# facebookresearch/NasRec

Measured on AMD Instinct MI355X. Metric: supernet samples/sec at batch 256 (Criteo-shape), 1/2/4/8 MI355X, higher is better.
Workload: dtype f32

## Files before the change

### nasrec_amd/csrc/gemm_rt.h

```cpp
#pragma once
#include <type_traits>
#include "gemm_tile.h"

struct RtStride {
  int R1, R0, K1, K0;
  bool kcontig;
};

__device__ __forceinline__ RtStride rt_stride(int mode, int ld) {
  if (mode == NASREC_AM_KC) return RtStride{16 * ld, ld, 16, 1, true};
  if (mode == NASREC_AM_RC) return RtStride{16, 1, 16 * ld, ld, false};
  if (mode == NASREC_AM_TOKR) return RtStride{ld, 1, 256, 16, false};
  return RtStride{256, 16, ld, 1, true};
}

__device__ __forceinline__ long rt_offset(const RtStride& s, int r, int k) {
  return (long)(r >> 4) * s.R1 + (long)(r & 15) * s.R0 + (long)(k >> 4) * s.K1 + (long)(k & 15) * s.K0;
}

template <bool KCONTIG, int NT, int TK, int R>
__device__ __forceinline__ void rt_stage_coords(int tid, int it, int& rr, int& kk) {
  if (KCONTIG) {
    kk = 4 * (tid & (TK / 4 - 1));
    rr = tid / (TK / 4) + (NT / (TK / 4)) * it;
  } else {
    rr = 4 * (tid & (R / 4 - 1));
    kk = tid / (R / 4) + (NT / (R / 4)) * it;
  }
}

__device__ __forceinline__ void rt_epilogue_store(int cm, const nasrec_gemm_desc_t& d, const nasrec_gemm_seg_t& sg, int i, int j, float v) {
  if (cm == NASREC_CM_PLAIN)
    epilogue_store<NASREC_CM_PLAIN>(d, sg, i, j, v);
  else
    epilogue_store<NASREC_CM_TOKJ>(d, sg, i, j, v);
}

__device__ __forceinline__ void rt_epilogue_store_col4(int cm, const nasrec_gemm_desc_t& d, const nasrec_gemm_seg_t& sg, int i0, int j, int M, const float (&v4)[4]) {
  if (cm == NASREC_CM_PLAIN)
    epilogue_store_col4<NASREC_CM_PLAIN>(d, sg, i0, j, M, v4);
  else
    epilogue_store_col4<NASREC_CM_TOKJ>(d, sg, i0, j, M, v4);
}

#define GEMM_RT_LDS_FLOATS(TBM, TBN, TK) (((TBM) + (TBN)) * ((TK) + 4) + 128)

template <bool KCA, bool KCB, int NT, int TK, int TBM, int TBN, bool AUX, int RING>
__device__ __forceinline__ void gemm_tile_rt(const nasrec_gemm_desc_t& d, int Mmax, int Nmax, const int bx, const int by, const int bz, float* lds) {
  const int AM = d.amode, BMODE = d.bmode, CM = d.cmode;
  constexpr int LDS_LD = TK + 4;
  constexpr int VA = 4, VB = 4;
  constexpr int NITA = TBM * TK / NT / VA, NITB = TBN * TK / NT / VB;
  static_assert((TBM * TK / NT) % VA == 0 && (TBN * TK / NT) % VB == 0 && TK % 16 == 0 && TBM % 4 == 0 && TBN % 4 == 0, "whole 16-byte pieces");
  constexpr int PER_WAVE = (TBM / 16) * (TBN / 16) / (NT / 64);
  constexpr int WTM = (PER_WAVE >= 2 && TBM >= 32) ? 32 : 16;
  constexpr int WTN = 16 * PER_WAVE / (WTM / 16);
  constexpr int FA = WTM / 16, FB = WTN / 16;
  static_assert(NITA >= 1 && NITB >= 1 && PER_WAVE >= 1 && (TBM / WTM) * (TBN / WTN) == NT / 64, "tile configuration");
  float* As = lds;
  float* Bs = lds + TBM * LDS_LD;
  const int tid = threadIdx.x;
  const int lane = tid & 63, wave = tid >> 6;
  const int wm = wave / (TBN / WTN), wn = wave % (TBN / WTN);
  const int fr = lane & 15, fg = lane >> 4;
  const int S = d.splitk > 1 ? d.splitk : 1;
  const int z = d.zmode ? bz / S : 0;
  const int ks = bz % S;
  const nasrec_gemm_seg_t& s0 = d.seg[z];
  const int M = s0.M, N = s0.N;
  const int m0 = by * TBM, n0 = bx * TBN;
  if (m0 >= M || n0 >= N) return;

  struct SegInfo {
    const float *A, *B, *Ax, *Bx;
    int K, lda, ldb, live;
  };
  static_assert(sizeof(SegInfo) * NASREC_MAX_SEGS <= 128 * sizeof(float), "segment table area");
  SegInfo* sinfo = reinterpret_cast<SegInfo*>(lds + (TBM + TBN) * LDS_LD);
  const bool use_table = !d.zmode && d.nseg > 1;
  if (use_table) {
    if (tid < d.nseg) {
      const nasrec_gemm_seg_t& sg = d.seg[tid];
      sinfo[tid] = SegInfo{sg.A, sg.B, sg.Aaux, sg.Baux, sg.K, sg.lda, sg.ldb, (sg.A != nullptr && sg.K > 0) ? 1 : 0};
    }
    __syncthreads();
  }
  int T = 0;
  if (!use_table) {
    T = (s0.A != nullptr && s0.K > 0) ? (s0.K + TK - 1) / TK : 0;
  } else {
    for (int q = 0; q < d.nseg; ++q)
      if (sinfo[q].live) T += (sinfo[q].K + TK - 1) / TK;
  }
  const int t0 = (int)((long)T * ks / S), t1 = (int)((long)T * (ks + 1) / S);

  f32x4 acc[FA][FB];
#pragma unroll
  for (int a = 0; a < FA; ++a)
#pragma unroll
    for (int b = 0; b < FB; ++b) acc[a][b] = (f32x4){0.f, 0.f, 0.f, 0.f};

  const int cOnes = s0.ones_col;
  const int Ra = (s0.Mvalid > 0 && s0.Mvalid < M) ? s0.Mvalid : M;
  const int Rb = cOnes ? N - 1 : N;
  const bool edgeA = (m0 + TBM > Ra), edgeB = (n0 + TBN > Rb);
  bool rvA[NITA], rvB[NITB];
  int kkA[NITA], kkB[NITB];
#pragma unroll
  for (int it = 0; it < NITA; ++it) {
    int rr;
    rt_stage_coords<KCA, NT, TK, TBM>(tid, it, rr, kkA[it]);
    rvA[it] = (m0 + rr) < Ra;
  }
#pragma unroll
  for (int it = 0; it < NITB; ++it) {
    int rr;
    rt_stage_coords<KCB, NT, TK, TBN>(tid, it, rr, kkB[it]);
    rvB[it] = (n0 + rr) < Rb;
  }

  int fs = z, fkt = t0;
  if (use_table) {
    fs = 0;
    int skip = t0;
    while (fs < d.nseg) {
      const int nt = sinfo[fs].live ? (sinfo[fs].K + TK - 1) / TK : 0;
      if (skip < nt) break;
      skip -= nt;
      ++fs;
    }
    fkt = skip;
  }
  const __amdgpu_buffer_rsrc_t rs_null = __builtin_amdgcn_make_buffer_rsrc(nullptr, 0, 0, 0x00020000);
  __amdgpu_buffer_rsrc_t rsA = rs_null, rsB = rs_null, rsAx = rs_null, rsBx = rs_null;
  bool hasAaux = false, hasBaux = false;
  int cK = 0, seg_tiles = 0;
  int stepA = 0, stepB = 0;
  unsigned voffA[NITA], voffB[NITB];
  unsigned koffA[NITA], koffB[NITB];
  auto load_seg = [&](int sq) {
    auto uptr = [](const float* p) -> const float* {
      const unsigned long long v = (unsigned long long)p;
      const unsigned lo = __builtin_amdgcn_readfirstlane((unsigned)v), hi = __builtin_amdgcn_readfirstlane((unsigned)(v >> 32));
      return (const float*)(((unsigned long long)hi << 32) | lo);
    };
    struct {
      const float *A, *B, *Aaux, *Baux;
      int K, lda, ldb;
    } sg;
    if (use_table) {
      sg = {uptr(sinfo[sq].A), uptr(sinfo[sq].B), uptr(sinfo[sq].Ax), uptr(sinfo[sq].Bx), __builtin_amdgcn_readfirstlane(sinfo[sq].K),
            __builtin_amdgcn_readfirstlane(sinfo[sq].lda), __builtin_amdgcn_readfirstlane(sinfo[sq].ldb)};
    } else {
      const nasrec_gemm_seg_t& g = d.seg[sq];
      sg = {g.A, g.B, g.Aaux, g.Baux, g.K, g.lda, g.ldb};
    }
    const int lda = sg.lda, ldb = sg.ldb;
    const RtStride sa_ = rt_stride(AM, lda), sb_ = rt_stride(BMODE, ldb);
    const int Rb_mem = cOnes ? N - 1 : N;
    const int extA = (M > 0 && sg.K > 0) ? (int)(4 * (rt_offset(sa_, M - 1, sg.K - 1) + 1)) : 0;
    const int extB = (Rb_mem > 0 && sg.K > 0) ? (int)(4 * (rt_offset(sb_, Rb_mem - 1, sg.K - 1) + 1)) : 0;
    rsA = __builtin_amdgcn_make_buffer_rsrc(const_cast<float*>(sg.A), 0, extA, 0x00020000);
    rsB = __builtin_amdgcn_make_buffer_rsrc(const_cast<float*>(sg.B), 0, extB, 0x00020000);
    hasAaux = AUX && sg.Aaux != nullptr;
    hasBaux = AUX && sg.Baux != nullptr;
    rsAx = hasAaux ? __builtin_amdgcn_make_buffer_rsrc(const_cast<float*>(sg.Aaux), 0, extA, 0x00020000) : rs_null;
    rsBx = hasBaux ? __builtin_amdgcn_make_buffer_rsrc(const_cast<float*>(sg.Baux), 0, extB, 0x00020000) : rs_null;
    cK = sg.K;
    seg_tiles = (cK + TK - 1) / TK;
    stepA = (int)(4 * rt_offset(sa_, 0, TK));
    stepB = (int)(4 * rt_offset(sb_, 0, TK));
#pragma unroll
    for (int it = 0; it < NITA; ++it) {
      int rr, kk;
      rt_stage_coords<KCA, NT, TK, TBM>(tid, it, rr, kk);
      koffA[it] = 4u * (unsigned)rt_offset(sa_, 0, kk);
      voffA[it] = 4u * (unsigned)rt_offset(sa_, rvA[it] ? m0 + rr : 0, kk);
    }
#pragma unroll
    for (int it = 0; it < NITB; ++it) {
      int rr, kk;
      rt_stage_coords<KCB, NT, TK, TBN>(tid, it, rr, kk);
      koffB[it] = 4u * (unsigned)rt_offset(sb_, 0, kk);
      voffB[it] = 4u * (unsigned)rt_offset(sb_, rvB[it] ? n0 + rr : 0, kk);
    }
  };

  float ra[RING][NITA][VA], rb[RING][NITB][VB];
  float xa[AUX ? RING : 1][AUX ? NITA : 1][VA], xb[AUX ? RING : 1][AUX ? NITB : 1][VB];
  auto stage_load = [](auto vtag, const __amdgpu_buffer_rsrc_t& rs, int voff, int soff, float* dst) {
    if (decltype(vtag)::value == 4) {
      const f32x4 t = __builtin_bit_cast(f32x4, __builtin_amdgcn_raw_buffer_load_b128(rs, voff, soff, 0));
      dst[0] = t[0], dst[1 % decltype(vtag)::value] = t[1], dst[2 % decltype(vtag)::value] = t[2], dst[3 % decltype(vtag)::value] = t[3];
    } else {
      dst[0] = __builtin_bit_cast(float, __builtin_amdgcn_raw_buffer_load_b32(rs, voff, soff, 0));
    }
  };
  using TagA = std::integral_constant<int, VA>;
  using TagB = std::integral_constant<int, VB>;
  int lim[RING];
  int fetched = t0;
  auto fetch = [&](int slot) {
    const bool live = fetched < t1;
    const int l = live ? cK - fkt * TK : 0;
    lim[slot] = l;
    const __amdgpu_buffer_rsrc_t ua = live ? rsA : rs_null, ub = live ? rsB : rs_null;
    const int sa = fkt * stepA, sb = fkt * stepB;
#pragma unroll
    for (int it = 0; it < NITA; ++it) {
      const int o = (int)((kkA[it] < l) ? voffA[it] : voffA[it] - koffA[it]);
      stage_load(TagA{}, ua, o, sa, ra[slot][it]);
      if (AUX) stage_load(TagA{}, live ? rsAx : rs_null, o, sa, xa[slot][it]);
    }
#pragma unroll
    for (int it = 0; it < NITB; ++it) {
      const int o = (int)((kkB[it] < l) ? voffB[it] : voffB[it] - koffB[it]);
      stage_load(TagB{}, ub, o, sb, rb[slot][it]);
      if (AUX) stage_load(TagB{}, live ? rsBx : rs_null, o, sb, xb[slot][it]);
    }
  };
  auto advance = [&]() {
    ++fetched;
    if (fetched >= t1) return;
    ++fkt;
    if (fkt >= seg_tiles) {
      if (use_table) {
        do {
          ++fs;
        } while (fs < d.nseg && !sinfo[fs].live);
        fkt = 0;
        load_seg(fs);
      }
    }
  };
  auto commit = [&](int slot) {
    const int l = lim[slot];
#pragma unroll
    for (int it = 0; it < NITA; ++it) {
      int rr, kk;
      rt_stage_coords<KCA, NT, TK, TBM>(tid, it, rr, kk);
      float a[VA];
#pragma unroll
      for (int e = 0; e < VA; ++e) {
        a[e] = ra[slot][it][e];
        if (AUX) a[e] = (!hasAaux || xa[slot][it][e] > 0.f) ? a[e] : 0.f;
        if (edgeA) a[e] = (m0 + rr + (KCA ? 0 : e) < Ra) ? a[e] : 0.f;
        a[e] = (kk + (KCA ? e : 0) < l) ? a[e] : 0.f;
      }
      if (KCA) {
        *reinterpret_cast<f32x4*>(&As[rr * LDS_LD + kk]) = (f32x4){a[0], a[1], a[2], a[3]};
      } else {
#pragma unroll
        for (int e = 0; e < VA; ++e) As[(rr + e) * LDS_LD + kk] = a[e];
      }
    }
#pragma unroll
    for (int it = 0; it < NITB; ++it) {
      int rr, kk;
      rt_stage_coords<KCB, NT, TK, TBN>(tid, it, rr, kk);
      float b[VB];
#pragma unroll
      for (int e = 0; e < VB; ++e) {
        b[e] = rb[slot][it][e];
        if (AUX) b[e] = (!hasBaux || xb[slot][it][e] > 0.f) ? b[e] : 0.f;
        if (edgeB) b[e] = (n0 + rr + (KCB ? 0 : e) < Rb) ? b[e] : 0.f;
        const bool kin = kk + (KCB ? e : 0) < l;
        b[e] = kin ? b[e] : 0.f;
        if (cOnes && (n0 + rr + (KCB ? 0 : e) == N - 1)) b[e] = kin ? 1.f : 0.f;
      }
      if (KCB) {
        *reinterpret_cast<f32x4*>(&Bs[rr * LDS_LD + kk]) = (f32x4){b[0], b[1], b[2], b[3]};
      } else {
#pragma unroll
        for (int e = 0; e < VB; ++e) Bs[(rr + e) * LDS_LD + kk] = b[e];
      }
    }
  };
  auto mfma_tile = [&]() {
#pragma unroll
    for (int kb = 0; kb < TK / 16; ++kb) {
      f32x4 af[FA], bf[FB];
#pragma unroll
      for (int a = 0; a < FA; ++a) af[a] = *reinterpret_cast<const f32x4*>(&As[(wm * WTM + a * 16 + fr) * LDS_LD + kb * 16 + 4 * fg]);
#pragma unroll
      for (int b = 0; b < FB; ++b) bf[b] = *reinterpret_cast<const f32x4*>(&Bs[(wn * WTN + b * 16 + fr) * LDS_LD + kb * 16 + 4 * fg]);
#pragma unroll
      for (int j = 0; j < 4; ++j)
#pragma unroll
        for (int a = 0; a < FA; ++a)
#pragma unroll
          for (int b = 0; b < FB; ++b) acc[a][b] = __builtin_amdgcn_mfma_f32_16x16x4f32(af[a][j], bf[b][j], acc[a][b], 0, 0, 0);
    }
  };

  if (t0 < t1) {
    load_seg(fs);
#pragma unroll
// ... 50 lines not shown
```

### nasrec_amd/csrc/worklist.hip

```cpp
#include <stdlib.h>
#include <string.h>

#include <vector>

#include "worklist_body.h"

static int wl_gemm_geometry(const nasrec_gemm_desc_t* g, nasrec_wl_item_t& it, int blob_left) {
  if (g->nseg < 1 || g->nseg > NASREC_MAX_SEGS) return nasrec_set_error(-2, "worklist: gemm nseg=%d", g->nseg);
  const int need = (int)offsetof(nasrec_gemm_desc_t, seg) + g->nseg * (int)sizeof(nasrec_gemm_seg_t);
  if (need > blob_left) return nasrec_set_error(-2, "worklist: truncated gemm descriptor (%d bytes) runs past the blob", need);
  const int nprob = g->zmode ? g->nseg : 1;
  const int S = g->splitk > 1 ? g->splitk : 1;
  if (g->splitk == NASREC_SPLITK_BALANCED) return nasrec_set_error(-2, "worklist: the balanced schedule is a throughput-regime launch");
  if ((it.part == 0) != (S == 1)) return nasrec_set_error(-2, "worklist: gemm part %d with splitk %d", it.part, g->splitk);
  if (S > 1 && !g->workspace) return nasrec_set_error(-3, "worklist: splitk=%d needs a workspace", S);
  int Mmax = 0, Nmax = 0, Kmax = 0;
  long wgs = 0;
  bool aux = false, uniform = true;
  for (int q = 0; q < nprob; ++q) {
    Mmax = g->seg[q].M > Mmax ? g->seg[q].M : Mmax;
    Nmax = g->seg[q].N > Nmax ? g->seg[q].N : Nmax;
    wgs += (long)((g->seg[q].M + 63) / 64) * ((g->seg[q].N + 63) / 64) * S;
  }
  for (int q = 0; q < g->nseg; ++q) {
    const nasrec_gemm_seg_t& s = g->seg[q];
    if (s.A && s.K > Kmax) Kmax = s.K;
    aux = aux || s.Aaux || s.Baux;
    if (!g->zmode && (s.ones_col != g->seg[0].ones_col || s.Mvalid != g->seg[0].Mvalid)) uniform = false;
    if (!g->zmode && s.A && ((s.Aaux != nullptr) != (g->seg[0].Aaux != nullptr) || (s.Baux != nullptr) != (g->seg[0].Baux != nullptr))) uniform = false;
  }
  if (!uniform) return nasrec_set_error(-2, "worklist: k-segments that disagree on row predicates / mask operands take the plain template");
  {
    const bool kca = g->amode == NASREC_AM_KC || g->amode == NASREC_AM_TOKK, kcb = g->bmode == NASREC_AM_KC || g->bmode == NASREC_AM_TOKK;
    if (!kca && kcb) return nasrec_set_error(-2, "worklist: operand binding a=%d b=%d has no body", g->amode, g->bmode);
  }
  if (Mmax <= 0 || Nmax <= 0) {
    it.nblk = 0;
    return 0;
  }
  if (it.part == 2) {
    const int per = (int)(((long)Mmax * Nmax + 255) / 256);
    it.geom[0] = per;
    it.nblk = per * nprob;
    return 0;
  }
  static const bool dense_body = getenv("NASREC_WL_DENSE_BODY") == nullptr || atoi(getenv("NASREC_WL_DENSE_BODY")) != 0;
  if (dense_body && it.part == 0 && !g->zmode && !aux && g->amode == NASREC_AM_KC && g->bmode == NASREC_AM_KC && g->cmode == NASREC_CM_PLAIN) {
    bool plain = true;
    int steps = 0;
    for (int q = 0; q < g->nseg; ++q) {
      const nasrec_gemm_seg_t& s = g->seg[q];
      plain = plain && !s.ones_col && !(s.Mvalid > 0 && s.Mvalid < Mmax);
      plain = plain && (long)Mmax * s.lda + s.K < (1L << 29) && (long)Nmax * s.ldb + s.K < (1L << 29);
      steps += (s.A && s.K > 0) ? (s.K + 15) >> 4 : 1;
    }
    if (plain && steps <= 2 * WL_DENSE_STEPS && (Mmax + 15) / 16 < 0x10000) {
      it.geom[0] = (Nmax + 15) / 16;
      it.geom[1] = (Mmax + 15) / 16 | (((steps + WL_DENSE_STEPS - 1) / WL_DENSE_STEPS) << 16);
      it.geom[2] = WL_TOKS | (3 << 2);
      it.nblk = (it.geom[0] * ((Mmax + 15) / 16) + 3) / 4;
      return 0;
    }
  }
  bool aux_b = false;
// ... 37 lines not shown
    for (int q = 0; q < g->nseg; ++q) {
      const nasrec_gemm_seg_t& s = g->seg[q];
      plain = plain && !s.ones_col && !(s.Mvalid > 0 && s.Mvalid < s.M) && s.N == Nmax && s.K <= 16 * WL_TOKDX_STEPS && s.M > 0;
      TU += (s.M + 15) / 16;
    }
    if (plain) {
      it.geom[0] = TU;
      it.geom[1] = 0;
      it.geom[2] = WL_TOKS | (2 << 2);
      it.nblk = std::min(((Nmax >> 4) * TU + 3) / 4, WL_TOK_MAX_WG);
      return 0;
    }
  }
  int tile, tbm, tbn;
  if (wgs >= GEMM_SKINNY_BELOW) {
    tile = WL_T32x32, tbm = 32, tbn = 32;
  } else {
    long pad64x16 = 0, pad16x64 = 0;
    for (int q = 0; q < nprob; ++q) {
      pad64x16 += (long)((g->seg[q].M + 63) / 64) * 64 * ((g->seg[q].N + 15) / 16) * 16;
      pad16x64 += (long)((g->seg[q].M + 15) / 16) * 16 * ((g->seg[q].N + 63) / 64) * 64;
    }
    static const bool by_padding = getenv("NASREC_WL_TILE_BY_PADDING") == nullptr || atoi(getenv("NASREC_WL_TILE_BY_PADDING")) != 0;
    const bool wide = by_padding && pad64x16 != pad16x64 ? pad64x16 < pad16x64 : Nmax >= Mmax;
    if (wide) {
      tile = WL_T64x16, tbm = 64, tbn = 16;
    } else {
      tile = WL_T16x64, tbm = 16, tbn = 64;
    }
  }
  it.geom[0] = (Nmax + tbn - 1) / tbn;
  it.geom[1] = (Mmax + tbm - 1) / tbm;
  const bool kca_ = g->amode == NASREC_AM_KC || g->amode == NASREC_AM_TOKK, kcb_ = g->bmode == NASREC_AM_KC || g->bmode == NASREC_AM_TOKK;
  it.geom[2] = tile | ((kca_ && kcb_ ? 0 : (kca_ ? 1 : 2)) << 2) | ((aux ? 1 : 0) << 4);
  it.nblk = it.geom[0] * it.geom[1] * nprob * S;
  return 0;
}

static int wl_item_geometry(nasrec_wl_item_t& it, const char* blob, int left, int k, bool& big) {
    it.nblk = 0;
    it.geom[0] = it.geom[1] = it.geom[2] = 0;
#define WL_NEED(T) if ((int)sizeof(T) > left) return nasrec_set_error(-2, "worklist: item %d runs past the blob", k)
    switch (it.kind) {
      case NASREC_OP_GEMM: {
        const int rc = wl_gemm_geometry(reinterpret_cast<const nasrec_gemm_desc_t*>(blob), it, left);
        if (rc) return rc;
        break;
      }
      case NASREC_OP_MHA_FWD:
      case NASREC_OP_MHA_BWD: {
        WL_NEED(nasrec_mha_desc_t);
        const nasrec_mha_desc_t* d = reinterpret_cast<const nasrec_mha_desc_t*>(blob);
        if (d->N < 1 || d->N > MHA_N) return nasrec_set_error(-2, "worklist: mha N=%d out of range [1,%d]", d->N, MHA_N);
        if (it.kind == NASREC_OP_MHA_BWD) {
          if (!d->saved) return nasrec_set_error(-2, "worklist: mha backward needs the state saved by the forward launch");
          big = true;
        }
        it.nblk = d->B;
        break;
      }
      case NASREC_OP_FM_FWD:
      case NASREC_OP_FM_BWD:
        WL_NEED(nasrec_fm_desc_t);
        it.nblk = (reinterpret_cast<const nasrec_fm_desc_t*>(blob)->B + 3) / 4;
        break;
      case NASREC_OP_DOT_TRI_FWD:
      case NASREC_OP_DOT_TRI_BWD: {
// ... 140 lines not shown
  if (!d->dev) return nasrec_set_error(-2, "worklist (device-resident): not prepared");
  if (d->total_blocks < 1) return 0;
  const unsigned* pf = d->pf;
  const unsigned* pm = d->pm;
  if (d->big) {
    hipLaunchKernelGGL(worklist_dev_kernel<true>, dim3((unsigned)d->total_blocks), dim3(256), sizeof(float) * WL_LDS_BIG_FLOATS, st, pf[0], pf[1], pf[2], pf[3],
                       pf[4], pf[5], pm[0], pm[1], pm[2], pm[3], pm[4], pm[5], d->dev);
  } else {
    hipLaunchKernelGGL(worklist_dev_kernel<false>, dim3((unsigned)d->total_blocks), dim3(256), sizeof(float) * WL_LDS_FLOATS, st, pf[0], pf[1], pf[2], pf[3],
                       pf[4], pf[5], pm[0], pm[1], pm[2], pm[3], pm[4], pm[5], d->dev);
  }
  return nasrec_check_launch("worklist (device-resident)");
}

#define PS_SPIN_BUDGET_TICKS 1000000ull

template <bool BIG>
__device__ __forceinline__ void ps_run_item(int it_kind, int it_part, int g0, int g1, int g2, unsigned long long blob, int vb, int nblk, int nwg) {
  float* lds = wl_lds;
  const int tid = threadIdx.x, wave = tid >> 6, lane = tid & 63;
  switch (it_kind) {
    case NASREC_OP_GEMM: {
      if (it_part == 2) {
        for (int u = vb; u < nblk; u += nwg) wl_gemm_second_pass(blob, u, g0);
        break;
      }
      const int cfg = g2;
      if ((cfg & 3) == WL_TOKS && ((cfg >> 2) & 3) == 3 && g1 == 0) wl_dense_small_dx(blob, vb, g0);
      else if ((cfg & 3) == WL_TOKS && ((cfg >> 2) & 3) == 3) wl_dense_small(blob, vb, g0, g1);
      else if ((cfg & 3) == WL_TOKS && ((cfg >> 2) & 3) == 1) wl_token_fwd(blob, vb, g0);
      else if ((cfg & 3) == WL_TOKS) wl_token_dx(blob, vb, g0);
      else if ((cfg >> 4) & 1) {
        for (int u = vb; u < nblk; u += nwg) {
          wl_gemm_bind<true>((cfg >> 2) & 3, cfg & 3, blob, u, g0, g1);
          if (u + nwg < nblk) __syncthreads();
        }
      } else {
        for (int u = vb; u < nblk; u += nwg) {
          wl_gemm_bind<false>((cfg >> 2) & 3, cfg & 3, blob, u, g0, g1);
          if (u + nwg < nblk) __syncthreads();
        }
      }
      break;
    }
    case NASREC_OP_MHA_FWD:
      wl_mha_fwd(blob, vb);
      break;
    case NASREC_OP_MHA_BWD:
      if (BIG) mha_bwd_tok(wl_ref<nasrec_mha_desc_t>(blob), __builtin_amdgcn_readfirstlane(vb), wl_lds);
      break;
    case NASREC_OP_FM_FWD: {
      const nasrec_fm_desc_t& d = wl_ref<nasrec_fm_desc_t>(blob);
      const int b = vb * 4 + wave;
      if (b < d.B) fm_fwd_sample(d, b, lane);
      break;
    }
    case NASREC_OP_FM_BWD: {
      const nasrec_fm_desc_t& d = wl_ref<nasrec_fm_desc_t>(blob);
      const int b = vb * 4 + wave;
      if (b < d.B) fm_bwd_sample(d, b, lane);
      break;
    }
    case NASREC_OP_DOT_TRI_FWD: {
      const nasrec_dot_tri_desc_t& d = wl_ref<nasrec_dot_tri_desc_t>(blob);
      const int b = vb * 4 + wave;
      if (b < d.B) dot_tri_fwd_sample(d, b, lane, lds + wave * (d.k1 * TRI_LD));
      break;
    }
    case NASREC_OP_DOT_TRI_BWD: {
      const nasrec_dot_tri_desc_t& d = wl_ref<nasrec_dot_tri_desc_t>(blob);
      const int b = vb * 4 + wave;
      const int P4 = (d.k1 * (d.k1 - 1) / 2 + 3) & ~3;
// ... 190 lines not shown
```

### nasrec_amd/csrc/worklist_body.h

```cpp
#pragma once
#include "attention_tok.h"
#include "gemm_rt.h"
#include "final_bodies.h"
#include "interact_bodies.h"
#include "dedup_bodies.h"

#define WL_LDS_BIG_FLOATS 9888
#define WL_LDS_FLOATS 7840
static_assert(MHA_TOK_BWD_LDS_FLOATS <= WL_LDS_BIG_FLOATS && MHA_TOK_FWD_LDS_FLOATS <= WL_LDS_FLOATS, "Transformer bodies fit the worklist launches");

#define WL_TK 64
#ifndef WL_AUX_RING2
#define WL_AUX_RING2 0
#endif
enum { WL_TOKS = 0, WL_T32x32 = 1, WL_T64x16 = 2, WL_T16x64 = 3 };

extern __shared__ __attribute__((aligned(16))) float wl_lds[];

template <typename T>
__device__ __forceinline__ const T& wl_ref(unsigned long long addr) {
  const unsigned lo = __builtin_amdgcn_readfirstlane((unsigned)addr), hi = __builtin_amdgcn_readfirstlane((unsigned)(addr >> 32));
  return *(const T*)(const __attribute__((address_space(4))) T*)(((unsigned long long)hi << 32) | lo);
}

template <bool KCA, bool KCB, int TBM, int TBN, bool AUX>
__device__ __forceinline__ void wl_gemm_cfg(unsigned long long blob, int vb_, int gx_, int gy_) {
  constexpr int RING = (AUX && !WL_AUX_RING2) ? 1 : 2;
  const nasrec_gemm_desc_t& g = wl_ref<nasrec_gemm_desc_t>(blob);
  const int vb = __builtin_amdgcn_readfirstlane(vb_), gx = __builtin_amdgcn_readfirstlane(gx_), gy = __builtin_amdgcn_readfirstlane(gy_);
  const int nprob = g.zmode ? g.nseg : 1;
  int Mmax = 0, Nmax = 0;
  for (int q = 0; q < nprob; ++q) {
    Mmax = max(Mmax, g.seg[q].M);
    Nmax = max(Nmax, g.seg[q].N);
  }
  const int bx = vb % gx, by = (vb / gx) % gy, bz = vb / (gx * gy);
  gemm_tile_rt<KCA, KCB, 256, WL_TK, TBM, TBN, AUX, RING>(g, Mmax, Nmax, bx, by, bz, wl_lds);
}

template <bool KCA, bool KCB, bool AUX>
__device__ __forceinline__ void wl_gemm_tile(int tile, unsigned long long off, int vb, int gx, int gy) {
  switch (tile) {
    case WL_T32x32: wl_gemm_cfg<KCA, KCB, 32, 32, AUX>(off, vb, gx, gy); break;
    case WL_T64x16: wl_gemm_cfg<KCA, KCB, 64, 16, AUX>(off, vb, gx, gy); break;
    default: wl_gemm_cfg<KCA, KCB, 16, 64, AUX>(off, vb, gx, gy); break;
  }
}

template <bool AUX>
__device__ __forceinline__ void wl_gemm_bind(int bind, int tile, unsigned long long off, int vb, int gx, int gy) {
  if (bind == 0) wl_gemm_tile<true, true, AUX>(tile, off, vb, gx, gy);
  else if (bind == 1) wl_gemm_tile<true, false, AUX>(tile, off, vb, gx, gy);
  else wl_gemm_tile<false, false, AUX>(tile, off, vb, gx, gy);
}

__device__ __forceinline__ void wl_warm_blob(unsigned long long addr, int bytes) {
  int sink, off;
  asm volatile(
      "s_mov_b32 %1, 0\n"
      "1:\n"
      "s_load_dword %0, %2, %1\n"
      "s_add_u32 %1, %1, 64\n"
      "s_cmp_lt_u32 %1, %3\n"
      "s_cbranch_scc1 1b\n"
      "s_waitcnt lgkmcnt(0)"
      : "=&s"(sink), "=&s"(off)
      : "s"(addr), "s"(bytes)
      : "scc", "memory");
}

#define WL_TOK_DEPTH 4
__device__ __forceinline__ void wl_token_fwd(unsigned long long blob, int vb_, int MT_) {
  const nasrec_gemm_desc_t& g = wl_ref<nasrec_gemm_desc_t>(blob);
  const int vb = __builtin_amdgcn_readfirstlane(vb_), MT = __builtin_amdgcn_readfirstlane(MT_);
  const int lane = threadIdx.x & 63, wave = __builtin_amdgcn_readfirstlane(threadIdx.x >> 6);
  const int e = lane & 15, fg = lane >> 4;
  wl_warm_blob(blob, (int)offsetof(nasrec_gemm_desc_t, seg) + g.nseg * (int)sizeof(nasrec_gemm_seg_t));
  const nasrec_gemm_seg_t& s0 = g.seg[0];
  const int M = s0.M, B = s0.N >> 4;
  const int unit = vb * 4 + wave;
  const int b = unit / MT, mt = unit - b * MT;
  if (b >= B) return;
  const int row = min(mt * 16 + e, M - 1);
  f32x4 acc = {0.f, 0.f, 0.f, 0.f};
  f32x4 fa[WL_TOK_DEPTH];
  float fb[WL_TOK_DEPTH][4];
// ... 275 lines not shown
    for (int q = 1; q < NASREC_WL_MAX_ITEMS; ++q) {
      const unsigned fq = (f[q >> 1] >> (16 * (q & 1))) & 0xffffu, mq = (m[q >> 1] >> (16 * (q & 1))) & 0xffffu;
      if ((unsigned)bid >= fq) {
        k = q;
        it_first = (int)fq;
        meta = mq;
      }
    }
    it_kind = meta & 63;
    it_part = (meta >> 6) & 3;
    it_off = (int)(meta >> 8) * 16;
  } else {
#pragma unroll 1
    while (k + 1 < wl.n && bid >= wl.item[k + 1].first) ++k;
    it_first = wl.item[k].first;
    it_kind = wl.item[k].kind;
    it_part = wl.item[k].part;
    it_off = wl.item[k].off;
  }
  const nasrec_wl_item_t& it = wl.item[k];
  const int vb = bid - it_first;
  const unsigned long long blob = base + offsetof(nasrec_worklist_desc_t, blob) + it_off;
  switch (it_kind) {
    case NASREC_OP_GEMM: {
      if (it_part == 2) {
        wl_gemm_second_pass(blob, vb, it.geom[0]);
        break;
      }
      const int cfg = it.geom[2];
      if ((cfg & 3) == WL_TOKS && ((cfg >> 2) & 3) == 3 && it.geom[1] == 0) wl_dense_small_dx(blob, vb, it.geom[0]);
      else if ((cfg & 3) == WL_TOKS && ((cfg >> 2) & 3) == 3) wl_dense_small(blob, vb, it.geom[0], it.geom[1]);
      else if ((cfg & 3) == WL_TOKS && ((cfg >> 2) & 3) == 1) wl_token_fwd(blob, vb, it.geom[0]);
      else if ((cfg & 3) == WL_TOKS) wl_token_dx(blob, vb, it.geom[0]);
      else if ((cfg >> 4) & 1) wl_gemm_bind<true>((cfg >> 2) & 3, cfg & 3, blob, vb, it.geom[0], it.geom[1]);
      else wl_gemm_bind<false>((cfg >> 2) & 3, cfg & 3, blob, vb, it.geom[0], it.geom[1]);
      break;
    }
    case NASREC_OP_MHA_FWD:
      wl_mha_fwd(blob, vb);
      break;
    case NASREC_OP_MHA_BWD:
      if (BIG) mha_bwd_tok(wl_ref<nasrec_mha_desc_t>(blob), __builtin_amdgcn_readfirstlane(vb), wl_lds);
      break;
    case NASREC_OP_FM_FWD: {
      const nasrec_fm_desc_t& d = wl_ref<nasrec_fm_desc_t>(blob);
      const int b = vb * 4 + wave;
      if (b < d.B) fm_fwd_sample(d, b, lane);
      break;
    }
    case NASREC_OP_FM_BWD: {
      const nasrec_fm_desc_t& d = wl_ref<nasrec_fm_desc_t>(blob);
      const int b = vb * 4 + wave;
      if (b < d.B) fm_bwd_sample(d, b, lane);
      break;
    }
    case NASREC_OP_DOT_TRI_FWD: {
      const nasrec_dot_tri_desc_t& d = wl_ref<nasrec_dot_tri_desc_t>(blob);
      const int b = vb * 4 + wave;
      if (b < d.B) dot_tri_fwd_sample(d, b, lane, lds + wave * (d.k1 * TRI_LD));
      break;
    }
    case NASREC_OP_DOT_TRI_BWD: {
      const nasrec_dot_tri_desc_t& d = wl_ref<nasrec_dot_tri_desc_t>(blob);
      const int b = vb * 4 + wave;
      const int P4 = (d.k1 * (d.k1 - 1) / 2 + 3) & ~3;
      if (b < d.B) dot_tri_bwd_sample(d, b, lane, lds + wave * (d.k1 * TRI_LD), lds + 4 * (d.k1 * TRI_LD) + wave * P4);
      break;
    }
// ... 45 lines not shown
```

### nasrec_amd/schedule.py

```python
import ctypes as C
import os
from typing import List, Tuple

from . import _lib as L

E = 16
MHA_PARAM_FLOATS = [768, 48, 256, 16, 16, 16, 256, 16, 256, 16, 16, 16]


class Acc:
    __slots__ = ("ptr", "width", "stride", "rows", "end")

    def __init__(self, ptr, rows, width_f, ld_f):
        self.ptr = int(ptr)
        self.rows = max(int(rows), 1)
        self.width = int(width_f) * 4
        self.stride = int(ld_f) * 4 if self.rows > 1 else self.width
        if self.stride < self.width:
            self.stride = self.width
        self.end = self.ptr + (self.rows - 1) * self.stride + self.width


def _flat(ptr, n_floats):
    return Acc(ptr, 1, n_floats, n_floats)
# ... 451 lines not shown


SOLO_TILES = int(os.environ.get("NASREC_WL_SOLO_TILES", "256"))


def gemm_capable(d) -> bool:
    if d.splitk == L.SPLITK_BALANCED or d.defer_second_pass or d.nseg < 1 or d.nseg > L.MAX_SEGS:
        return False
    kca, kcb = d.amode in (L.AM_KC, L.AM_TOKK), d.bmode in (L.AM_KC, L.AM_TOKK)
    if not kca and kcb:
        return False
    if d.splitk > 1 and not d.workspace:
        return False
    nprob = d.nseg if d.zmode else 1
    S = d.splitk if d.splitk > 1 else 1
    if nprob == 1 and ((d.seg[0].M + 63) // 64) * ((d.seg[0].N + 63) // 64) * S >= SOLO_TILES:
        return False
    if not getattr(d, "_wl_force", False):
        from . import plan as P
        one = d
        if d.splitk > 1:
            one = L.GemmDesc.from_buffer_copy(d)
            one.splitk = 1
        if P.gemm_route(one)[1] & (1 << L.GEMM_ROUTE_KSLICE):
            return False
    s0 = d.seg[0]
    if not d.zmode:
        for q in range(d.nseg):
            s = d.seg[q]
            if s.ones_col != s0.ones_col or s.Mvalid != s0.Mvalid:
                return False
            if s.A and (bool(s.Aaux) != bool(s0.Aaux) or bool(s.Baux) != bool(s0.Baux)):
                return False
    return True


def item_bytes(node):
    d = node.desc
    k = d.kind
    if isinstance(d, L.GemmDesc):
        if not gemm_capable(d):
            return None
        if (node.part == "whole") != (d.splitk <= 1):
            return None
        return C.string_at(C.addressof(d), _GEMM_HEAD + d.nseg * _SEG_BYTES)
    if k in (L.OP_DOT_TRI_FWD, L.OP_DOT_TRI_BWD):
        P4 = (d.k1 * (d.k1 - 1) // 2 + 3) & ~3
        if d.k1 < 2 or 4 * (d.k1 * 20 + P4) > WL_LDS_FLOATS:
            return None
    if k in (L.OP_MHA_FWD, L.OP_MHA_BWD) and (d.N < 1 or d.N > 64 or (k == L.OP_MHA_BWD and not d.saved)):
        return None
    if k == L.OP_DEDUP_IDS and (d.B < 1 or d.B > 256 or d.cap != 256 or d.Fs < 1 or d.Fs > L.MAX_TABLES
                                or not (d.idx and d.leader and d.order and d.lists and d.counts)):
        return None
    if k == L.OP_FINAL_FUSED and (not (d.y and d.logits and d.bias and d.w) or d.nsplit > 1 or any(d.dseg[q] and not d.seg[q] for q in range(d.nseg))):
        return None
    if k == L.OP_FINAL_BWD and d.y and not d.logits:
        return None
    if k in _PLAIN_KINDS:
        return C.string_at(C.addressof(d), C.sizeof(d))
    if k == L.OP_REDUCE_ROWS and 1 <= d.ndst <= L.WL_REDUCE_DST:
        r = L.WlReduce()
        r.kind, r.R, r.C, r.ld, r.in_, r.ndst = d.kind, d.R, d.C, d.ld, d.in_, d.ndst
        for q in range(d.ndst):
            r.dst[q], r.dst_off[q], r.dst_len[q] = d.dst[q], d.dst_off[q], d.dst_len[q]
        return C.string_at(C.addressof(r), C.sizeof(r))
# ... 292 lines not shown
```

Before: 1.162 million.

## Specialize worklist GEMM mask staging per side and compress per-thread offsets

Replaces the boolean AUX template flag with a per-operand mask selector, so worklist GEMM items stage only the one mask operand they actually have. Items with masks on both sides fall back to the plain template. Mask items now run with a two-deep load ring instead of one. Per-iteration offset arrays are replaced by a base row offset plus a constant per-iteration stride, and the thread index is masked so the compiler can bound it. The aim is lower VGPR pressure and more prefetch depth in the masked GEMM path, at the cost of more template instantiations and code size.

```diff
diff --git a/nasrec_amd/csrc/gemm_rt.h b/nasrec_amd/csrc/gemm_rt.h
--- a/nasrec_amd/csrc/gemm_rt.h
+++ b/nasrec_amd/csrc/gemm_rt.h
@@ -45,7 +45,9 @@
 
 #define GEMM_RT_LDS_FLOATS(TBM, TBN, TK) (((TBM) + (TBN)) * ((TK) + 4) + 128)
 
-template <bool KCA, bool KCB, int NT, int TK, int TBM, int TBN, bool AUX, int RING>
+enum { RT_MASK_NONE = 0, RT_MASK_A = 1, RT_MASK_B = 2, RT_MASK_BOTH = 3 };
+
+template <bool KCA, bool KCB, int NT, int TK, int TBM, int TBN, int MASK, int RING>
 __device__ __forceinline__ void gemm_tile_rt(const nasrec_gemm_desc_t& d, int Mmax, int Nmax, const int bx, const int by, const int bz, float* lds) {
   const int AM = d.amode, BMODE = d.bmode, CM = d.cmode;
   constexpr int LDS_LD = TK + 4;
@@ -59,7 +61,10 @@
   static_assert(NITA >= 1 && NITB >= 1 && PER_WAVE >= 1 && (TBM / WTM) * (TBN / WTN) == NT / 64, "tile configuration");
   float* As = lds;
   float* Bs = lds + TBM * LDS_LD;
-  const int tid = threadIdx.x;
+  unsigned tid_ = threadIdx.x;
+  asm volatile("" : "+v"(tid_));
+  const int tid = (int)(tid_ & 255u);
+  static_assert(NT <= 256 && (NT & (NT - 1)) == 0, "thread index mask");
   const int lane = tid & 63, wave = tid >> 6;
   const int wm = wave / (TBN / WTN), wn = wave % (TBN / WTN);
   const int fr = lane & 15, fg = lane >> 4;
@@ -105,19 +110,21 @@
   const int Rb = cOnes ? N - 1 : N;
   const bool edgeA = (m0 + TBM > Ra), edgeB = (n0 + TBN > Rb);
   bool rvA[NITA], rvB[NITB];
-  int kkA[NITA], kkB[NITB];
 #pragma unroll
   for (int it = 0; it < NITA; ++it) {
-    int rr;
-    rt_stage_coords<KCA, NT, TK, TBM>(tid, it, rr, kkA[it]);
+    int rr, kk;
+    rt_stage_coords<KCA, NT, TK, TBM>(tid, it, rr, kk);
     rvA[it] = (m0 + rr) < Ra;
   }
 #pragma unroll
   for (int it = 0; it < NITB; ++it) {
-    int rr;
-    rt_stage_coords<KCB, NT, TK, TBN>(tid, it, rr, kkB[it]);
+    int rr, kk;
+    rt_stage_coords<KCB, NT, TK, TBN>(tid, it, rr, kk);
     rvB[it] = (n0 + rr) < Rb;
   }
+  constexpr int DRA = KCA ? NT / (TK / 4) : 0, DKA = KCA ? 0 : NT / (TBM / 4);
+  constexpr int DRB = KCB ? NT / (TK / 4) : 0, DKB = KCB ? 0 : NT / (TBN / 4);
+  static_assert(DRA % 16 == 0 && DKA % 16 == 0 && DRB % 16 == 0 && DKB % 16 == 0 && TBM % 16 == 0 && TBN % 16 == 0, "whole blocks between a thread's loads");
 
   int fs = z, fkt = t0;
   if (use_table) {
@@ -136,8 +143,9 @@
   bool hasAaux = false, hasBaux = false;
   int cK = 0, seg_tiles = 0;
   int stepA = 0, stepB = 0;
-  unsigned voffA[NITA], voffB[NITB];
-  unsigned koffA[NITA], koffB[NITB];
+  unsigned rowA = 0, rowB = 0;
+  unsigned kofA = 0, kofB = 0;
+  int itA = 0, itB = 0;
   auto load_seg = [&](int sq) {
     auto uptr = [](const float* p) -> const float* {
       const unsigned long long v = (unsigned long long)p;
@@ -162,32 +170,43 @@
     const int extB = (Rb_mem > 0 && sg.K > 0) ? (int)(4 * (rt_offset(sb_, Rb_mem - 1, sg.K - 1) + 1)) : 0;
     rsA = __builtin_amdgcn_make_buffer_rsrc(const_cast<float*>(sg.A), 0, extA, 0x00020000);
     rsB = __builtin_amdgcn_make_buffer_rsrc(const_cast<float*>(sg.B), 0, extB, 0x00020000);
-    hasAaux = AUX && sg.Aaux != nullptr;
-    hasBaux = AUX && sg.Baux != nullptr;
+    hasAaux = (MASK & RT_MASK_A) && sg.Aaux != nullptr;
+    hasBaux = (MASK & RT_MASK_B) && sg.Baux != nullptr;
     rsAx = hasAaux ? __builtin_amdgcn_make_buffer_rsrc(const_cast<float*>(sg.Aaux), 0, extA, 0x00020000) : rs_null;
     rsBx = hasBaux ? __builtin_amdgcn_make_buffer_rsrc(const_cast<float*>(sg.Baux), 0, extB, 0x00020000) : rs_null;
     cK = sg.K;
     seg_tiles = (cK + TK - 1) / TK;
     stepA = (int)(4 * rt_offset(sa_, 0, TK));
     stepB = (int)(4 * rt_offset(sb_, 0, TK));
-#pragma unroll
-    for (int it = 0; it < NITA; ++it) {
+    {
       int rr, kk;
-      rt_stage_coords<KCA, NT, TK, TBM>(tid, it, rr, kk);
-      koffA[it] = 4u * (unsigned)rt_offset(sa_, 0, kk);
-      voffA[it] = 4u * (unsigned)rt_offset(sa_, rvA[it] ? m0 + rr : 0, kk);
-    }
-#pragma unroll
-    for (int it = 0; it < NITB; ++it) {
-      int rr, kk;
-      rt_stage_coords<KCB, NT, TK, TBN>(tid, it, rr, kk);
-      koffB[it] = 4u * (unsigned)rt_offset(sb_, 0, kk);
-      voffB[it] = 4u * (unsigned)rt_offset(sb_, rvB[it] ? n0 + rr : 0, kk);
-    }
+      rt_stage_coords<KCA, NT, TK, TBM>(tid, 0, rr, kk);
+      rowA = 4u * (unsigned)rt_offset(sa_, m0 + rr, 0);
+      kofA = 4u * (unsigned)rt_offset(sa_, 0, kk);
+      itA = (int)(4 * rt_offset(sa_, DRA, DKA));
+      rt_stage_coords<KCB, NT, TK, TBN>(tid, 0, rr, kk);
+      rowB = 4u * (unsigned)rt_offset(sb_, n0 + rr, 0);
+      kofB = 4u * (unsigned)rt_offset(sb_, 0, kk);
+      itB = (int)(4 * rt_offset(sb_, DRB, DKB));
+    }
+  };
+  auto offA = [&](int it, int l) -> int {
+    int rr, kk;
+    rt_stage_coords<KCA, NT, TK, TBM>(tid, it, rr, kk);
+    const unsigned r = rvA[it] ? rowA + (KCA ? (unsigned)(it * itA) : 0u) : 0u;
+    const unsigned k = kk < l ? kofA + (KCA ? 0u : (unsigned)(it * itA)) : 0u;
+    return (int)(r + k);
+  };
+  auto offB = [&](int it, int l) -> int {
+    int rr, kk;
+    rt_stage_coords<KCB, NT, TK, TBN>(tid, it, rr, kk);
+    const unsigned r = rvB[it] ? rowB + (KCB ? (unsigned)(it * itB) : 0u) : 0u;
+    const unsigned k = kk < l ? kofB + (KCB ? 0u : (unsigned)(it * itB)) : 0u;
+    return (int)(r + k);
   };
 
   float ra[RING][NITA][VA], rb[RING][NITB][VB];
-  float xa[AUX ? RING : 1][AUX ? NITA : 1][VA], xb[AUX ? RING : 1][AUX ? NITB : 1][VB];
+  float xa[(MASK & RT_MASK_A) ? RING : 1][(MASK & RT_MASK_A) ? NITA : 1][VA], xb[(MASK & RT_MASK_B) ? RING : 1][(MASK & RT_MASK_B) ? NITB : 1][VB];
   auto stage_load = [](auto vtag, const __amdgpu_buffer_rsrc_t& rs, int voff, int soff, float* dst) {
     if (decltype(vtag)::value == 4) {
       const f32x4 t = __builtin_bit_cast(f32x4, __builtin_amdgcn_raw_buffer_load_b128(rs, voff, soff, 0));
@@ -208,15 +227,15 @@
     const int sa = fkt * stepA, sb = fkt * stepB;
 #pragma unroll
     for (int it = 0; it < NITA; ++it) {
-      const int o = (int)((kkA[it] < l) ? voffA[it] : voffA[it] - koffA[it]);
+      const int o = offA(it, l);
       stage_load(TagA{}, ua, o, sa, ra[slot][it]);
-      if (AUX) stage_load(TagA{}, live ? rsAx : rs_null, o, sa, xa[slot][it]);
+      if (MASK & RT_MASK_A) stage_load(TagA{}, live ? rsAx : rs_null, o, sa, xa[slot][it]);
     }
 #pragma unroll
     for (int it = 0; it < NITB; ++it) {
-      const int o = (int)((kkB[it] < l) ? voffB[it] : voffB[it] - koffB[it]);
+      const int o = offB(it, l);
       stage_load(TagB{}, ub, o, sb, rb[slot][it]);
-      if (AUX) stage_load(TagB{}, live ? rsBx : rs_null, o, sb, xb[slot][it]);
+      if (MASK & RT_MASK_B) stage_load(TagB{}, live ? rsBx : rs_null, o, sb, xb[slot][it]);
     }
   };
   auto advance = [&]() {
@@ -243,7 +262,7 @@
 #pragma unroll
       for (int e = 0; e < VA; ++e) {
         a[e] = ra[slot][it][e];
-        if (AUX) a[e] = (!hasAaux || xa[slot][it][e] > 0.f) ? a[e] : 0.f;
+        if (MASK & RT_MASK_A) a[e] = (!hasAaux || xa[slot][it][e] > 0.f) ? a[e] : 0.f;
         if (edgeA) a[e] = (m0 + rr + (KCA ? 0 : e) < Ra) ? a[e] : 0.f;
         a[e] = (kk + (KCA ? e : 0) < l) ? a[e] : 0.f;
       }
@@ -262,7 +281,7 @@
 #pragma unroll
       for (int e = 0; e < VB; ++e) {
         b[e] = rb[slot][it][e];
-        if (AUX) b[e] = (!hasBaux || xb[slot][it][e] > 0.f) ? b[e] : 0.f;
+        if (MASK & RT_MASK_B) b[e] = (!hasBaux || xb[slot][it][e] > 0.f) ? b[e] : 0.f;
         if (edgeB) b[e] = (n0 + rr + (KCB ? 0 : e) < Rb) ? b[e] : 0.f;
         const bool kin = kk + (KCB ? e : 0) < l;
         b[e] = kin ? b[e] : 0.f;
diff --git a/nasrec_amd/csrc/worklist.hip b/nasrec_amd/csrc/worklist.hip
--- a/nasrec_amd/csrc/worklist.hip
+++ b/nasrec_amd/csrc/worklist.hip
@@ -17,6 +17,7 @@
   int Mmax = 0, Nmax = 0, Kmax = 0;
   long wgs = 0;
   bool aux = false, uniform = true;
+  bool mask_a = false, mask_b = false;
   for (int q = 0; q < nprob; ++q) {
     Mmax = g->seg[q].M > Mmax ? g->seg[q].M : Mmax;
     Nmax = g->seg[q].N > Nmax ? g->seg[q].N : Nmax;
@@ -26,10 +27,13 @@
     const nasrec_gemm_seg_t& s = g->seg[q];
     if (s.A && s.K > Kmax) Kmax = s.K;
     aux = aux || s.Aaux || s.Baux;
+    mask_a = mask_a || s.Aaux;
+    mask_b = mask_b || s.Baux;
     if (!g->zmode && (s.ones_col != g->seg[0].ones_col || s.Mvalid != g->seg[0].Mvalid)) uniform = false;
     if (!g->zmode && s.A && ((s.Aaux != nullptr) != (g->seg[0].Aaux != nullptr) || (s.Baux != nullptr) != (g->seg[0].Baux != nullptr))) uniform = false;
   }
   if (!uniform) return nasrec_set_error(-2, "worklist: k-segments that disagree on row predicates / mask operands take the plain template");
+  if (mask_a && mask_b) return nasrec_set_error(-2, "worklist: mask operands on both sides (an item stages ONE mask copy) take the plain template");
   {
     const bool kca = g->amode == NASREC_AM_KC || g->amode == NASREC_AM_TOKK, kcb = g->bmode == NASREC_AM_KC || g->bmode == NASREC_AM_TOKK;
     if (!kca && kcb) return nasrec_set_error(-2, "worklist: operand binding a=%d b=%d has no body", g->amode, g->bmode);
@@ -133,7 +137,7 @@
   it.geom[0] = (Nmax + tbn - 1) / tbn;
   it.geom[1] = (Mmax + tbm - 1) / tbm;
   const bool kca_ = g->amode == NASREC_AM_KC || g->amode == NASREC_AM_TOKK, kcb_ = g->bmode == NASREC_AM_KC || g->bmode == NASREC_AM_TOKK;
-  it.geom[2] = tile | ((kca_ && kcb_ ? 0 : (kca_ ? 1 : 2)) << 2) | ((aux ? 1 : 0) << 4);
+  it.geom[2] = tile | ((kca_ && kcb_ ? 0 : (kca_ ? 1 : 2)) << 2) | ((aux ? 1 : 0) << 4) | ((mask_b ? 1 : 0) << 5);
   it.nblk = it.geom[0] * it.geom[1] * nprob * S;
   return 0;
 }
@@ -340,12 +344,12 @@
       else if ((cfg & 3) == WL_TOKS) wl_token_dx(blob, vb, g0);
       else if ((cfg >> 4) & 1) {
         for (int u = vb; u < nblk; u += nwg) {
-          wl_gemm_bind<true>((cfg >> 2) & 3, cfg & 3, blob, u, g0, g1);
+          wl_gemm_bind<RT_MASK_BOTH, 1>((cfg >> 2) & 3, cfg & 3, blob, u, g0, g1);
           if (u + nwg < nblk) __syncthreads();
         }
       } else {
         for (int u = vb; u < nblk; u += nwg) {
-          wl_gemm_bind<false>((cfg >> 2) & 3, cfg & 3, blob, u, g0, g1);
+          wl_gemm_bind<RT_MASK_NONE>((cfg >> 2) & 3, cfg & 3, blob, u, g0, g1);
           if (u + nwg < nblk) __syncthreads();
         }
       }
diff --git a/nasrec_amd/csrc/worklist_body.h b/nasrec_amd/csrc/worklist_body.h
--- a/nasrec_amd/csrc/worklist_body.h
+++ b/nasrec_amd/csrc/worklist_body.h
@@ -10,9 +10,6 @@
 static_assert(MHA_TOK_BWD_LDS_FLOATS <= WL_LDS_BIG_FLOATS && MHA_TOK_FWD_LDS_FLOATS <= WL_LDS_FLOATS, "Transformer bodies fit the worklist launches");
 
 #define WL_TK 64
-#ifndef WL_AUX_RING2
-#define WL_AUX_RING2 0
-#endif
 enum { WL_TOKS = 0, WL_T32x32 = 1, WL_T64x16 = 2, WL_T16x64 = 3 };
 
 extern __shared__ __attribute__((aligned(16))) float wl_lds[];
@@ -23,9 +20,8 @@
   return *(const T*)(const __attribute__((address_space(4))) T*)(((unsigned long long)hi << 32) | lo);
 }
 
-template <bool KCA, bool KCB, int TBM, int TBN, bool AUX>
+template <bool KCA, bool KCB, int TBM, int TBN, int MASK, int RING>
 __device__ __forceinline__ void wl_gemm_cfg(unsigned long long blob, int vb_, int gx_, int gy_) {
-  constexpr int RING = (AUX && !WL_AUX_RING2) ? 1 : 2;
   const nasrec_gemm_desc_t& g = wl_ref<nasrec_gemm_desc_t>(blob);
   const int vb = __builtin_amdgcn_readfirstlane(vb_), gx = __builtin_amdgcn_readfirstlane(gx_), gy = __builtin_amdgcn_readfirstlane(gy_);
   const int nprob = g.zmode ? g.nseg : 1;
@@ -35,23 +31,23 @@
     Nmax = max(Nmax, g.seg[q].N);
   }
   const int bx = vb % gx, by = (vb / gx) % gy, bz = vb / (gx * gy);
-  gemm_tile_rt<KCA, KCB, 256, WL_TK, TBM, TBN, AUX, RING>(g, Mmax, Nmax, bx, by, bz, wl_lds);
-}
-
-template <bool KCA, bool KCB, bool AUX>
+  gemm_tile_rt<KCA, KCB, 256, WL_TK, TBM, TBN, MASK, RING>(g, Mmax, Nmax, bx, by, bz, wl_lds);
+}
+
+template <bool KCA, bool KCB, int MASK, int RING>
 __device__ __forceinline__ void wl_gemm_tile(int tile, unsigned long long off, int vb, int gx, int gy) {
   switch (tile) {
-    case WL_T32x32: wl_gemm_cfg<KCA, KCB, 32, 32, AUX>(off, vb, gx, gy); break;
-    case WL_T64x16: wl_gemm_cfg<KCA, KCB, 64, 16, AUX>(off, vb, gx, gy); break;
-    default: wl_gemm_cfg<KCA, KCB, 16, 64, AUX>(off, vb, gx, gy); break;
-  }
-}
-
-template <bool AUX>
+    case WL_T32x32: wl_gemm_cfg<KCA, KCB, 32, 32, MASK, RING>(off, vb, gx, gy); break;
+    case WL_T64x16: wl_gemm_cfg<KCA, KCB, 64, 16, MASK, RING>(off, vb, gx, gy); break;
+    default: wl_gemm_cfg<KCA, KCB, 16, 64, MASK, RING>(off, vb, gx, gy); break;
+  }
+}
+
+template <int MASK, int RING = 2>
 __device__ __forceinline__ void wl_gemm_bind(int bind, int tile, unsigned long long off, int vb, int gx, int gy) {
-  if (bind == 0) wl_gemm_tile<true, true, AUX>(tile, off, vb, gx, gy);
-  else if (bind == 1) wl_gemm_tile<true, false, AUX>(tile, off, vb, gx, gy);
-  else wl_gemm_tile<false, false, AUX>(tile, off, vb, gx, gy);
+  if (bind == 0) wl_gemm_tile<true, true, MASK, RING>(tile, off, vb, gx, gy);
+  else if (bind == 1) wl_gemm_tile<true, false, MASK, RING>(tile, off, vb, gx, gy);
+  else wl_gemm_tile<false, false, MASK, RING>(tile, off, vb, gx, gy);
 }
 
 __device__ __forceinline__ void wl_warm_blob(unsigned long long addr, int bytes) {
@@ -393,8 +389,9 @@
       else if ((cfg & 3) == WL_TOKS && ((cfg >> 2) & 3) == 3) wl_dense_small(blob, vb, it.geom[0], it.geom[1]);
       else if ((cfg & 3) == WL_TOKS && ((cfg >> 2) & 3) == 1) wl_token_fwd(blob, vb, it.geom[0]);
       else if ((cfg & 3) == WL_TOKS) wl_token_dx(blob, vb, it.geom[0]);
-      else if ((cfg >> 4) & 1) wl_gemm_bind<true>((cfg >> 2) & 3, cfg & 3, blob, vb, it.geom[0], it.geom[1]);
-      else wl_gemm_bind<false>((cfg >> 2) & 3, cfg & 3, blob, vb, it.geom[0], it.geom[1]);
+      else if (((cfg >> 4) & 3) == 3) wl_gemm_bind<RT_MASK_B>((cfg >> 2) & 3, cfg & 3, blob, vb, it.geom[0], it.geom[1]);
+      else if ((cfg >> 4) & 1) wl_gemm_bind<RT_MASK_A>((cfg >> 2) & 3, cfg & 3, blob, vb, it.geom[0], it.geom[1]);
+      else wl_gemm_bind<RT_MASK_NONE>((cfg >> 2) & 3, cfg & 3, blob, vb, it.geom[0], it.geom[1]);
       break;
     }
     case NASREC_OP_MHA_FWD:
diff --git a/nasrec_amd/schedule.py b/nasrec_amd/schedule.py
--- a/nasrec_amd/schedule.py
+++ b/nasrec_amd/schedule.py
@@ -507,6 +507,8 @@
                 return False
             if s.A and (bool(s.Aaux) != bool(s0.Aaux) or bool(s.Baux) != bool(s0.Baux)):
                 return False
+    if any(d.seg[q].Aaux for q in range(d.nseg)) and any(d.seg[q].Baux for q in range(d.nseg)):
+        return False
     return True
 
 
```

Result: no change. 1.160 million (-0.2%).
